# leavesnight/VIEO_SLAM

Measured on AMD Instinct MI355X. Metric: frontend+localBA frames/sec on EuRoC MH05 stereo-VIO; ATE vs ref, higher is better.
Workload: dtype u8 (extract/match) + f64 (pose optimisation)

## Files before the change

### vieo_slam_amd/csrc/lba.hip

```cpp
#include <atomic>
#include <chrono>
#include <mutex>
#include <thread>
#include <vector>

#include "gba_sparse_plan.h"
#include "imu_device.h"
#include "rccl_dl.h"

namespace vieo {

struct LbaKf {
  double p[3], qw, qx, qy, qz;
  int col;
  int fixed;
  double v[3], dbg[3], dba[3], bg[3], ba[3];
};

struct LbaImu {
  int i, j;
  int has_imu, robust;
  double InfoI[81];
  double infoBg, infoBa;
  vieo_imu_preint M;
// ... 29 lines not shown
  int np, n_free, npv;
  int pd;
  int n_imu;
  const LbaImu* imu;
  const int *kf_in, *kf_out;
  double* Ae;
  double *gchi0, *gchi;
  double* bfull;
  double* red;
  double* red_sc;
  const unsigned char* close;
  double thMono, thMonoClose, thStereo;
  double gw[3];
  double th_dist_far;
  double qRbe[4], pbe[3];
  int ldS;
  int* kf_list;
  int* kf_act;
  const int *kf_edge_first, *kf_edge_idx;
  int* tab;
  LbaKf *kf, *kf_bak;
  double *X, *X_bak;
  double* err;
  unsigned char *level, *erase, *mp_act;
  const int *mp_first, *mp_count;
  double* CB;
  double* Bs;
  double* Sp;
  size_t sp_stride;
  int ksplit;
  double *Hll, *bl, *Hpp, *bp, *Hs, *bs, *xp;
  unsigned char* occ;
  int use_occ;
  double *Hb, *Wp;
  int* big_fail;
  int nb;
  double *part0, *part, *part_m, *pmax;
  double* part_t;
  int* tail_cnt;
  int n_chunks;
  int fold_kernel;
  int *chunk_first, *chunk_kf;
  int* chunk_cnt;
  double* chunk_part;
  CamD cam;
  CamD cams[4];
  int n_cams;
  const unsigned char* ocam;
  double dMono, dStereo;
  int solver;
  int scale_opt;
  double* scl;
  double* sc_sys;
  double* psc;
  const int *sch_ptr, *sch_i, *sch_j, *sch_diag, *sch_off;
  int n_sch_diag, n_sch_off;
  const int *col_ptr, *tile_i, *tile_j;
  const int *row_ptr, *row_j, *row_tile;
  const int *upd_ptr, *upd;
  int nt, n_tiles;
};

__device__ __forceinline__ double win_scale(const LbaDev& D) { return D.scale_opt ? D.scl[0] : 1.0; }
__device__ __forceinline__ void scaled_point(const LbaDev& D, int m, double* Xs) {
  const double s = win_scale(D);
  Xs[0] = D.X[3 * (size_t)m] * s, Xs[1] = D.X[3 * (size_t)m + 1] * s, Xs[2] = D.X[3 * (size_t)m + 2] * s;
// ... 653 lines not shown
  }
  if (threadIdx.x == 0) out[w].lambda = 1e-5 * s_m[0];
}

typedef double double4_t __attribute__((ext_vector_type(4)));
static const int kChunkLm = 16, kLd = 3 * kChunkLm + 2;
#ifndef VIEO_SCHUR_AB
#define VIEO_SCHUR_AB 0
#endif

__global__ void __launch_bounds__(256)
k_lba_occ(const LbaDev* __restrict__ devs, const WinCtl* __restrict__ ctl) {
  const int w = blockIdx.y;
  if (!(ctl[w].flags & LBA_BEGIN)) return;
  const LbaDev& D = devs[w];
  if (!D.use_occ) return;
  const int np = D.npv, CB = (np + 64) >> 6, nchunks = (D.n_mp + kChunkLm - 1) / kChunkLm;
  const int e = blockIdx.x * 256 + threadIdx.x;
  if (np == 0 || e >= CB * nchunks) return;
  const int bi = e / nchunks, ch = e - bi * nchunks;
  const int a0 = bi * 64 / 6, a1 = min((bi * 64 + 63) / 6, D.n_free - 1);
  int any = D.scale_opt && (np - 1) >= bi * 64 && (np - 1) < bi * 64 + 64;
  for (int a = a0; a <= a1 && !any; a++)
    for (int j = 0; j < kChunkLm; j++) {
      const int m = ch * kChunkLm + j;
      if (m < D.n_mp && D.tab[(size_t)a * D.n_mp + m] >= 0) {
        any = 1;
        break;
      }
    }
  D.occ[e] = (unsigned char)any;
}

template <bool OFFDIAG, bool TILES = false>
__global__ void __launch_bounds__(256, OFFDIAG ? 2 : 3)
k_lba_schur(const LbaDev* __restrict__ devs, const WinCtl* __restrict__ ctl, const WinOut* __restrict__ out) {
  __shared__ __attribute__((aligned(16))) double sT[64 * kLd];
  __shared__ __attribute__((aligned(16))) double sB[64 * kLd];
  __shared__ double sDi[2][kChunkLm * 9];
  const int w = blockIdx.y;
  if (!(ctl[w].flags & LBA_TRIAL)) return;
  const LbaDev& D = devs[w];
  const int np = D.npv;
  if (np == 0) return;
  const int RB = (np + 63) >> 6, CB = (np + 64) >> 6;
  const int ksplit = D.ksplit;
  int bt = blockIdx.x / ksplit;
  const int split = blockIdx.x % ksplit;
  int bi = 0, bj;
  if (TILES != (D.solver == 3)) return;
  if (TILES) {
    if (bt >= (OFFDIAG ? D.n_sch_off : D.n_sch_diag)) return;
    bt = (OFFDIAG ? D.sch_off : D.sch_diag)[bt];
    bi = D.sch_i[bt], bj = D.sch_j[bt];
  } else if (OFFDIAG) {
    while (bi < RB && bt >= CB - bi - 1) bt -= CB - bi - 1, bi++;
    if (bi >= RB) return;
    bj = bi + 1 + bt;
  } else {
    if (bt >= RB) return;
    bi = bj = bt;
  }
  const int nchunks = (D.n_mp + kChunkLm - 1) / kChunkLm, cps = (nchunks + ksplit - 1) / ksplit;
  const int c0 = split * cps, c1 = min(nchunks, c0 + cps);
  if (c0 >= c1) return;
  const double lambda = win_lambda(ctl[w], out[w]);
  const int tid = threadIdx.x, lane = tid & 63;
  const int wv = __builtin_amdgcn_readfirstlane(tid >> 6);
  const int n_mp = D.n_mp;
  double4_t acc[4];
#pragma unroll
  for (int q = 0; q < 4; q++) acc[q] = (double4_t){0, 0, 0, 0};
  const unsigned char* occ_i = D.occ + (size_t)bi * nchunks;
  const unsigned char* occ_j = D.occ + (size_t)bj * nchunks;
  const bool has_bl = np >= bj * 64 && np < bj * 64 + 64;
  const bool use_occ = D.use_occ != 0;
  auto next_chunk = [&](int ch) {
    if (use_occ)
      while (ch < c1 && (!occ_i[ch] || (!has_bl && !occ_j[ch]))) ch++;
    return ch;
  };
  typedef double dbl2_t __attribute__((ext_vector_type(2)));
  typedef const dbl2_t __attribute__((address_space(1)))* gd2p;
  typedef const double __attribute__((address_space(1)))* gdp;
  typedef const int __attribute__((address_space(1)))* gip;
  typedef const unsigned char __attribute__((address_space(1)))* gbp;
  const gd2p gCB = (gd2p)D.CB;
  const gdp gBs = (gdp)D.Bs, gbl = (gdp)D.bl, gHll = (gdp)D.Hll;
  const gip gtab = (gip)D.tab;
  const gbp gact = (gbp)D.mp_act;
  const int ps = tid >> 4, pj = tid & 15;
  const int nfree = D.n_free, n_obs = D.n_obs;
  const bool sc_opt = D.scale_opt != 0;
  constexpr bool offdiag = OFFDIAG;
  const int aT = (64 * bi) / 6 + ps, aB = (64 * bj) / 6 + ps;
// ... 40 lines not shown
    if (lane < kChunkLm) {
#pragma unroll
      for (int t = 0; t < 9; t++) sDi[buf][lane * 9 + t] = hl_on ? Di[t] : 0.0;
    }
  };
  auto stage_T = [&](const double* v, const double* Di) {
    const double d0 = Di[0], d1 = Di[1], d2 = Di[2], d3 = Di[3], d4 = Di[4], d5 = Di[5], d6 = Di[6], d7 = Di[7], d8 = Di[8];
#pragma unroll
    for (int q = 0; q < 6; q++) {
      const unsigned r = (unsigned)(rT + q);
      if (r < 64u) {
        double b0 = v[3 * q], b1 = v[3 * q + 1], b2 = v[3 * q + 2];
        if (q == 0) b0 += spT3[0], b1 += spT3[1], b2 += spT3[2];
        double* d = sT + r * kLd + 3 * pj;
        d[0] = __builtin_fma(b2, d6, __builtin_fma(b1, d3, b0 * d0));
        d[1] = __builtin_fma(b2, d7, __builtin_fma(b1, d4, b0 * d1));
        d[2] = __builtin_fma(b2, d8, __builtin_fma(b1, d5, b0 * d2));
      }
    }
  };
  auto stage_B = [&](const double* v, const double* sp) {
#pragma unroll
    for (int q = 0; q < 6; q++) {
      const unsigned r = (unsigned)(rB + q);
      if (r < 64u) {
        double* d = sB + r * kLd + 3 * pj;
        double b0 = v[3 * q], b1 = v[3 * q + 1], b2 = v[3 * q + 2];
        if (q == 0) b0 += sp[0], b1 += sp[1], b2 += sp[2];
        if (q < 2 && (q == 1) == sc_opt) b0 += blv[0], b1 += blv[1], b2 += blv[2];
        d[0] = b0, d[1] = b1, d[2] = b2;
      }
    }
  };
#ifdef VIEO_SCHUR_PROBE
  long long tp[6] = {0, 0, 0, 0, 0, 0}, t0 = __builtin_readcyclecounter(), t1;
#define SCHUR_TICK(i) t1 = __builtin_readcyclecounter(), tp[i] += t1 - t0, t0 = t1;
#else
#define SCHUR_TICK(i)
#endif
  int ch = next_chunk(c0), buf = 0;
  int nx = ch < c1 ? next_chunk(ch + 1) : c1;
  int nx2 = nx < c1 ? next_chunk(nx + 1) : c1;
  int eT = -1, eB = -1;
  if (wv < 3) {
    load_blk(tab_of(aT, aTc, ch), ta);
    if (offdiag) load_blk(tab_of(aB, aBc, ch), tb);
    if (spT) load_special(aT, ch, !offdiag, spT3, blv);
    if (offdiag && spB) load_special(aB, ch, true, spB3, blv);
    eT = tab_of(aT, aTc, nx);
    if (offdiag) eB = tab_of(aB, aBc, nx);
  } else {
    load_hll(ch);
    store_dinv(0);
    load_hll(nx);
  }
  while (ch < c1) {
    __syncthreads();
    SCHUR_TICK(0)
    if (wv < 3) {
      if (!(VIEO_SCHUR_AB & 2)) {
        stage_T(ta, sDi[buf] + pj * 9);
        if (offdiag)
          stage_B(tb, spB3);
        else
          stage_B(ta, spT3);
      }
    } else {
      store_dinv(buf ^ 1);
      load_hll(nx2);
    }
    SCHUR_TICK(1)
    __syncthreads();
    SCHUR_TICK(2)
    const int nx3 = nx2 < c1 ? next_chunk(nx2 + 1) : c1;
    if (wv < 3 && nx < c1) {
      load_blk(eT, ta);
      if (offdiag) load_blk(eB, tb);
      if (spT) load_special(aT, nx, !offdiag, spT3, blv);
      if (offdiag && spB) load_special(aB, nx, true, spB3, blv);
      eT = tab_of(aT, aTc, nx2);
      if (offdiag) eB = tab_of(aB, aBc, nx2);
    }
    SCHUR_TICK(3)
    {
      const double* pa = sT + (wv * 16 + (lane & 15)) * kLd + (lane >> 4);
      const double* pb = sB + (lane & 15) * kLd + (lane >> 4);
#if !(VIEO_SCHUR_AB & 1)
#pragma unroll
      for (int ks = 0; ks < 3 * kChunkLm / 4; ks++) {
        const double av = pa[ks * 4];
#pragma unroll
        for (int q = 0; q < 4; q++)
          acc[q] = __builtin_amdgcn_mfma_f64_16x16x4f64(av, pb[q * 16 * kLd + ks * 4], acc[q], 0, 0, 0);
      }
#else
      acc[0][0] += pa[0] + pb[0];
#endif
    }
    SCHUR_TICK(4)
    buf ^= 1, ch = nx, nx = nx2, nx2 = nx3;
  }
#ifdef VIEO_SCHUR_PROBE
  if ((blockIdx.x == 3 || blockIdx.x == 40) && (blockIdx.y == 0 || blockIdx.y == 3) && (tid == 0 || tid == 64 || tid == 200))
    printf("schur probe w %d bx %d tid %d tile (%d,%d) chunks %d: wait_A %lld stage %lld wait_B %lld issue_loads %lld mfma %lld\n",
           w, (int)blockIdx.x, tid, bi, bj, c1 - c0, tp[0], tp[1], tp[2], tp[3], tp[4]);
#endif
  double* S = D.Sp + (size_t)split * D.sp_stride;
  if (TILES) {
    S += (size_t)bt * kGbaTileElems;
#pragma unroll
    for (int q = 0; q < 4; q++)
#pragma unroll
      for (int r = 0; r < 4; r++) S[(wv * 16 + (lane >> 4) + 4 * r) * 64 + q * 16 + (lane & 15)] = acc[q][r];
    return;
  }
#pragma unroll
  for (int q = 0; q < 4; q++)
#pragma unroll
    for (int r = 0; r < 4; r++)
      S[(size_t)(bi * 64 + wv * 16 + (lane >> 4) + 4 * r) * D.ldS + bj * 64 + q * 16 + (lane & 15)] = acc[q][r];
}

__global__ void __launch_bounds__(256)
k_lba_pack(const LbaDev* __restrict__ devs, const WinCtl* __restrict__ ctl) {
  const int w = blockIdx.y;
  if (!(ctl[w].flags & LBA_TRIAL)) return;
  const LbaDev& D = devs[w];
  if (!D.red) return;
  const int npv = D.npv, nS = npv * (npv + 1), nH = 36 * D.n_free, nb = 6 * D.n_free;
  const int e = blockIdx.x * 256 + threadIdx.x;
  if (e >= nS + nH + nb + (D.scale_opt ? nb + 2 : 0)) return;
  if (e < nS) {
    const int ksplit = D.ksplit;
    const int nchunks = (D.n_mp + kChunkLm - 1) / kChunkLm, cps = (nchunks + ksplit - 1) / ksplit;
    const int ns = (nchunks + cps - 1) / cps;
    const int r = e / (npv + 1), c = e - r * (npv + 1);
    const int rr = c < npv ? min(r, c) : r, cc = c < npv ? max(r, c) : npv;
    double s = 0;
    for (int k = 0; k < ns; k++) s += D.Sp[(size_t)k * D.sp_stride + (size_t)rr * D.ldS + cc];
    D.red[e] = s;
  } else if (e < nS + nH)
    D.red[e] = D.Hpp[e - nS];
  else if (e < nS + nH + nb)
    D.red[e] = D.bp[e - nS - nH];
  else
    D.red[e] = D.sc_sys[e - nS - nH - nb];
}

// ... 1543 lines not shown
    o.scl = take(16);
    H.o_kf = o.kf, H.o_X = o.X, H.o_erase = o.erase, H.o_scl = o.scl;
  }
  const size_t res_end = arena;
  for (int w = 0; w < W; w++) {
    const WinHost& H = win[w];
    if (H.skip) continue;
    off[w].level = take(H.n_obs), off[w].err = take((size_t)H.n_obs * 24);
  }
  const size_t zero_end = arena;
  if ((rc = g_stage.ensure(res_end)) != VIEO_OK) return rc;
  uint8_t* hs = (uint8_t*)g_stage.p;
  int max_obs = 0, max_mp = 0, max_kf = 0, max_nf = 0, max_imu = 0, max_chunks = 1;
  bool any_multicam = false;
  for (int w = 0; w < W; w++) {
    if (win[w].skip) continue;
    max_nf = std::max(max_nf, win[w].nf), max_mp = std::max(max_mp, win[w].n_mp);
  }
  const int cps_target = 8;
  auto schur_tiles = [&](int nf) {
    const int npm = 6 * nf + sco, RB = (npm + 63) / 64, CB = (npm + 64) / 64;
    return RB * CB - RB * (RB - 1) / 2;
  };
  auto schur_ksplit = [&](int nf, int nmp) {
    const int nch = (nmp + kChunkLm - 1) / kChunkLm, nbt = std::max(1, schur_tiles(nf));
    if (gba) return std::max(1, std::min(std::min(nch, 16), 768 / nbt));
    return std::max(1, std::min(std::min((nch + cps_target - 1) / cps_target, 32), std::max(1, 512 / nbt)));
  };
  int schur_grid = 0, schur_grid_off = 0;
  int schur_grid_t = 0, schur_grid_t_off = 0;
  std::vector<size_t> scratch_off(W);
  struct Scr {
    size_t kf_bak, X_bak, mp_act, BB, Bs, Sp, Hll, bl, Hpp, Hs, bp, bs, xp, part0, part, part_m, pmax, kf_list, tab, Ae, gchi0,
        gchi, bfull, Hb, Wp, big_fail, kf_act, occ, sc_sys, psc, part_t, tail_cnt, chunk_first, chunk_kf, chunk_cnt, chunk_part;
    int nb;
  };
  std::vector<Scr> scr(W);
  for (int w = 0; w < W; w++) {
    WinHost& H = win[w];
    if (H.skip) continue;
    const int nf = H.nf;
    Scr& s = scr[w];
    const int npm = 6 * nf + sco;
    s.kf_bak = take((size_t)H.n_kf * sizeof(LbaKf)), s.X_bak = take((size_t)H.n_mp * 24);
    s.mp_act = take(H.n_mp);
    const int sp_rows = (npm + 63) / 64 * 64, ldS = (npm + 64) / 64 * 64;
    s.BB = take(((size_t)H.n_obs + 1) * 144);
    s.Bs = sco ? take((size_t)std::max(H.n_mp, 1) * 24) : 0;
    const int ksplit = schur_ksplit(nf, H.n_mp);
    const bool tiles = wcls[w] == 3;
    const GbaSparsePlan& PL = plans[w];
    if (tiles) {
      schur_grid_t = std::max(schur_grid_t, (int)PL.sch_diag.size() * ksplit);
      schur_grid_t_off = std::max(schur_grid_t_off, (int)PL.sch_off.size() * ksplit);
    } else {
      const int RBw = (npm + 63) / 64;
      schur_grid = std::max(schur_grid, RBw * ksplit);
      schur_grid_off = std::max(schur_grid_off, (schur_tiles(nf) - RBw) * ksplit);
    }
    s.Sp = take(tiles ? PL.schur_bytes(ksplit) : (size_t)ksplit * sp_rows * ldS * 8);
    s.Hll = take((size_t)H.n_mp * 72), s.bl = take((size_t)H.n_mp * 24);
    const int npf = pd * nf + sco;
    s.Hpp = take((size_t)std::max(nf, 1) * 36 * 8), s.Hs = tiles ? 0 : take((size_t)npf * npf * 8);
    s.nb = (npf + 1 + kNB - 1) / kNB * kNB;
    s.Hb = s.Wp = s.big_fail = 0;
    if (tiles) {
      s.Hb = take(PL.pool_bytes()), s.Wp = take(PL.panel_bytes()), s.big_fail = take(256);
    } else if (wcls[w] == 2) {
      s.Hb = take((size_t)s.nb * s.nb * 8), s.Wp = take((size_t)s.nb * kNB * 8), s.big_fail = take(256);
    } else if (wcls[w] == 1) {
      s.nb = (npf + 16) >> 4;
      s.Hb = take(ldg_scratch_doubles(s.nb) * 8);
    }
    s.bp = take((size_t)npm * 8), s.bs = take((size_t)npf * 8), s.xp = take((size_t)npf * 8);
    s.bfull = take((size_t)npf * 8);
    s.Ae = take((size_t)std::max(H.n_imu, 1) * 930 * 8);
    s.gchi0 = take((size_t)std::max(H.n_imu, 1) * 8), s.gchi = take((size_t)std::max(H.n_imu, 1) * 8);
    s.part0 = take((size_t)((H.n_obs + 255) / 256) * 8), s.part = take((size_t)((H.n_obs + 255) / 256) * 8);
    s.part_m = take((size_t)((H.n_mp + 63) / 64) * 8), s.pmax = take((size_t)((H.n_mp + 63) / 64) * 8);
    s.part_t = take((size_t)std::max((H.n_mp + 63) / 64, 1) * 8), s.tail_cnt = take(256);
    {
      const size_t nchk = (size_t)H.n_obs / kBuildChunk + nf + 1;
      s.chunk_first = take((size_t)(nf + 1) * 4), s.chunk_cnt = take((size_t)(nf + 1) * 4);
      s.chunk_kf = take(nchk * 4), s.chunk_part = take(nchk * 33 * 8);
      max_chunks = std::max(max_chunks, (int)nchk);
    }
    s.kf_list = take((size_t)H.n_kf * 4), s.tab = take((size_t)std::max(nf, 1) * H.n_mp * 4);
    s.sc_sys = take((size_t)(6 * nf + 2) * 8), s.psc = take((size_t)((H.n_mp + 63) / 64) * 16);
    s.kf_act = take((size_t)H.n_kf * 4);
    s.occ = take((size_t)((npm + 64) / 64) * ((H.n_mp + kChunkLm - 1) / kChunkLm));
    LbaDev& D = devs[w];
    memset(&D, 0, sizeof(D));
    D.n_obs = H.n_obs, D.n_mp = H.n_mp, D.n_kf = H.n_kf, D.nf_cap = nf;
    D.ldS = ldS, D.sp_stride = tiles ? PL.n_sch_tiles() * kGbaTileElems : (size_t)sp_rows * ldS, D.ksplit = ksplit;
    D.cam.fx = H.P->fx, D.cam.fy = H.P->fy, D.cam.cx = H.P->cx, D.cam.cy = H.P->cy, D.cam.bf = H.P->bf;
    memcpy(D.cam.Rcb, H.P->Rcb, 72);
    memcpy(D.cam.tcb, H.P->tcb, 24);
    D.n_cams = H.P->n_cams;
    any_multicam |= H.P->n_cams > 0;
    for (int ci = 0; ci < H.P->n_cams; ci++) {
      const vieo_camera& c = H.P->cams[ci];
      CamD& d = D.cams[ci];
      d.fx = c.fx, d.fy = c.fy, d.cx = c.cx, d.cy = c.cy, d.bf = 0;
      memcpy(d.Rcb, c.Rcb, 72), memcpy(d.tcb, c.tcb, 24);
      d.model = c.model, d.num_k = c.model == VIEO_CAM_RADTAN ? c.num_k : 0;
      for (int q = 0; q < 8; q++) d.k[q] = (double)c.dist[q];
    }
    D.dMono = (double)(float)sqrt(gba ? 5.99 : 5.991), D.dStereo = (double)(float)sqrt(7.815);
    D.pd = pd, D.n_imu = H.n_imu;
    D.scale_opt = sco;
    D.use_occ = gba ? 1 : 0;
    D.solver = wcls[w];
    if (tiles) {
      D.n_sch_diag = (int)PL.sch_diag.size(), D.n_sch_off = (int)PL.sch_off.size();
      D.nt = PL.nt, D.n_tiles = (int)PL.n_tiles();
    }
    if (vio) {
      D.thMono = (double)5.991f, D.thMonoClose = 1.5 * (double)5.991f, D.thStereo = 7.815;
      memcpy(D.gw, H.VP->gw, 24);
      memcpy(D.qRbe, H.VP->qRbe, 32), memcpy(D.pbe, H.VP->pbe, 24);
      D.th_dist_far = (!gba && H.VP->th_dist_far > 0 && std::isfinite(H.VP->th_dist_far)) ? (double)H.VP->th_dist_far : 0.0;
      H.prelevel_pending = !gba;
    } else {
// ... 171 lines not shown
      g_lba_sparse_stats[0] = (long long)P.n_tiles(), g_lba_sparse_stats[1] = (long long)P.nt * (P.nt + 1) / 2;
      g_lba_sparse_stats[2] = (long long)P.n_sch_tiles(), g_lba_sparse_stats[3] = (long long)P.vrb * P.vcb - (long long)P.vrb * (P.vrb - 1) / 2;
      g_lba_sparse_stats[4] = (long long)P.bytes(devs[w].ksplit), g_lba_sparse_stats[5] = (long long)arena;
    }
  if ((rc = g_small.ensure(small_bytes)) != VIEO_OK) return rc;
  if ((rc = g_small_h.ensure((size_t)W * (sizeof(WinCtl) + sizeof(WinOut) + 32))) != VIEO_OK) return rc;
  uint8_t* base = g_arena.as<uint8_t>();
  for (int w = 0; w < W; w++) {
    if (win[w].skip) continue;
    const Off& o = off[w];
    const Scr& s = scr[w];
    LbaDev& D = devs[w];
    D.obs = (const vieo_lba_obs*)(base + o.obs);
    D.mp_first = (const int*)(base + o.mp_first), D.mp_count = (const int*)(base + o.mp_count);
    D.kf_edge_first = (const int*)(base + o.kf_edge_first), D.kf_edge_idx = (const int*)(base + o.kf_edge_idx);
    D.kf = (LbaKf*)(base + o.kf), D.X = (double*)(base + o.X), D.erase = base + o.erase;
    D.level = base + o.level, D.err = (double*)(base + o.err);
    D.ocam = base + o.ocam;
    D.kf_bak = (LbaKf*)(base + s.kf_bak), D.X_bak = (double*)(base + s.X_bak), D.mp_act = base + s.mp_act;
    D.CB = (double*)(base + s.BB), D.Bs = (double*)(base + s.Bs), D.Sp = (double*)(base + s.Sp);
    D.Hll = (double*)(base + s.Hll), D.bl = (double*)(base + s.bl);
    D.Hpp = (double*)(base + s.Hpp), D.Hs = (double*)(base + s.Hs), D.bp = (double*)(base + s.bp);
    D.Hb = (double*)(base + s.Hb), D.Wp = (double*)(base + s.Wp), D.big_fail = (int*)(base + s.big_fail);
    D.nb = s.nb;
    D.bs = (double*)(base + s.bs), D.xp = (double*)(base + s.xp);
    D.part0 = (double*)(base + s.part0), D.part = (double*)(base + s.part);
    D.part_m = (double*)(base + s.part_m), D.pmax = (double*)(base + s.pmax);
    D.part_t = (double*)(base + s.part_t), D.tail_cnt = (int*)(base + s.tail_cnt);
    D.fold_kernel = W <= 4 ? 0 : 1;
    D.chunk_first = (int*)(base + s.chunk_first), D.chunk_cnt = (int*)(base + s.chunk_cnt);
    D.chunk_kf = (int*)(base + s.chunk_kf), D.chunk_part = (double*)(base + s.chunk_part);
    D.kf_list = (int*)(base + s.kf_list), D.tab = (int*)(base + s.tab);
    D.kf_act = (int*)(base + s.kf_act), D.occ = base + s.occ;
    D.bfull = (double*)(base + s.bfull), D.Ae = (double*)(base + s.Ae);
    D.gchi0 = (double*)(base + s.gchi0), D.gchi = (double*)(base + s.gchi);
    D.scl = (double*)(base + o.scl), D.sc_sys = (double*)(base + s.sc_sys), D.psc = (double*)(base + s.psc);
    if (vio || win[w].ENC) {
      D.imu = (const LbaImu*)(base + o.imu), D.close = base + o.close;
      D.kf_in = (const int*)(base + o.kf_in), D.kf_out = (const int*)(base + o.kf_out);
    }
    if (wcls[w] == 3) {
      const int* d = (const int*)(base + o.plan);
      for (auto& l : plan_lists(plans[w], &D)) *l.second = d, d += l.first->size();
    }
  }
  size_t shard_sys = 0;
  if (sh) {
    for (int w = 0; w < W; w++) {
      if (win[w].skip) continue;
      devs[w].red = sh->d_buf + shard_sys;
      shard_sys += shard_sys_doubles(devs[w].nf_cap, sco);
    }
    if (shard_sys + 4 * (size_t)W > sh->cap) {
      set_error("sharded local BA: reduction buffer too small (%zu doubles needed)", shard_sys + 4 * (size_t)W);
      return VIEO_E_CAPACITY;
    }
    for (int w = 0; w < W; w++) devs[w].red_sc = sh->d_buf + shard_sys + 4 * (size_t)w;
  }
  LbaDev* dD = g_small.as<LbaDev>();
  WinCtl* dC = (WinCtl*)(dD + W);
  WinOut* dO = (WinOut*)(dC + W);
  int* dWins = (int*)(dO + W);
  WinCtl* ctl = (WinCtl*)g_small_h.p;
  WinOut* out = (WinOut*)(ctl + W);
  double* h_sc = (double*)(out + W);
  const double ms_described = ms_since(t_enter);
// ... 79 lines not shown
          H.stage = 2;
        else if (H.stage == 0 && !stop_now) {
          f |= LBA_CLASS0;
          H.stage = 1, H.iters = H.P->its1, H.phase = H.iters > 0 ? 0 : 2;
        } else {
          if (H.stage == 0) H.R->status = VIEO_LBA_ABORTED;
          f |= LBA_CLASS1;
          H.stage = 2;
        }
      }
      if (H.stage < 2 && H.phase == 0) {
        f |= LBA_BEGIN | LBA_BUILD | LBA_TRIAL | ((gba ? gba->robust != 0 : H.stage == 0) ? LBA_ROBUST : 0);
        lam = vio && !gba ? H.VP->lambda_init : -1;
        if (H.prelevel_pending) f |= LBA_PRELEVEL, H.prelevel_pending = false;
      } else if (H.stage < 2 && H.phase == 1) {
        f |= LBA_TRIAL | ((gba ? gba->robust != 0 : H.stage == 0) ? LBA_ROBUST : 0);
        if (H.need_build) f |= LBA_BUILD;
        if (H.need_restore) f |= LBA_RESTORE, H.need_restore = false;
      }
      ctl[w].flags = f, ctl[w].pad = sh ? stop_req : 0, ctl[w].lambda = lam;
      any |= f;
      if ((f & LBA_TRIAL) && !H.skip) cls_trial[devs[w].solver] = true;
    }
    if (!any) break;
    VIEO_HIP_CHECK(hipMemcpyAsync(dC, ctl, (size_t)W * sizeof(WinCtl), hipMemcpyHostToDevice, st));
    if (any & LBA_RESTORE) KT.launch(KC_OTHER, [&] { hipLaunchKernelGGL(k_lba_restore, dim3(gr, W), dim3(256), 0, st, dD, dC); });
    if (any & (LBA_CLASS0 | LBA_CLASS1)) KT.launch(KC_OTHER, [&] { hipLaunchKernelGGL(k_lba_classify, dim3(ge, W), dim3(256), 0, st, dD, dC); });
    if (any & LBA_PRELEVEL)
      for (int ph = 0; ph < 3; ph++) KT.launch(KC_OTHER, [&] { hipLaunchKernelGGL(k_lba_prelevel, dim3(ge, W), dim3(256), 0, st, dD, dC, ph); });
    if (any & LBA_BEGIN) {
      KT.launch(KC_BEGIN, [&] { hipLaunchKernelGGL(k_lba_zero, dim3(64, W), dim3(256), 0, st, dD, dC); });
      KT.launch(KC_BEGIN, [&] { hipLaunchKernelGGL(k_lba_begin, dim3(W), dim3(1024), 0, st, dD, dC, dO); });
      if (gba) KT.launch(KC_BEGIN, [&] { hipLaunchKernelGGL(k_lba_occ, dim3(std::max(1, (occ_max + 255) / 256), W), dim3(256), 0, st, dD, dC); });
      KT.launch(KC_ERROR, [&] { hipLaunchKernelGGL(k_lba_error, dim3(ge, W), dim3(256), 0, st, dD, dC, 0); });
    }
    if (any & LBA_BUILD) {
      auto build2 = [&](auto mc, auto sc) {
        constexpr bool MC = decltype(mc)::value, SC = decltype(sc)::value;
        if (fused_build) {
          KT.launch(KC_BUILD, [&] { hipLaunchKernelGGL((k_lba_build<MC, SC, 2>), dim3(gq + max_chunks + max_imu, W), dim3(256), 0, st, dD, dC, max_chunks, gq); });
          if (W > 4) KT.launch(KC_BUILD, [&] { hipLaunchKernelGGL(k_lba_build_fold, dim3(std::max(1, max_nf), W), dim3(64), 0, st, dD, dC); });
          return;
        }
        KT.launch(KC_BUILD, [&] { hipLaunchKernelGGL((k_lba_build<MC, SC, 0>), dim3(gq, W), dim3(256), 0, st, dD, dC, 0, 0); });
        KT.launch(KC_BUILD, [&] { hipLaunchKernelGGL((k_lba_build<MC, SC, 1>), dim3(max_chunks, W), dim3(256), 0, st, dD, dC, max_chunks, 0); });
        if (W > 4) KT.launch(KC_BUILD, [&] { hipLaunchKernelGGL(k_lba_build_fold, dim3(std::max(1, max_nf), W), dim3(64), 0, st, dD, dC); });
      };
      if (sco) {
        if (any_multicam)
          build2(std::true_type(), std::true_type());
        else
          build2(std::false_type(), std::true_type());
        KT.launch(KC_BUILD, [&] { hipLaunchKernelGGL(k_lba_scale_fold, dim3(W), dim3(256), 0, st, dD, dC); });
      } else if (any_multicam)
        build2(std::true_type(), std::false_type());
      else
        build2(std::false_type(), std::false_type());
      if (!fused_build && max_imu > 0) KT.launch(KC_GENERIC, [&] { hipLaunchKernelGGL(k_lba_generic, dim3(max_imu, W), dim3(64), 0, st, dD, dC, 0); });
    }
    if (any & LBA_BEGIN) KT.launch(KC_BEGIN, [&] { hipLaunchKernelGGL(k_lba_lambda, dim3(W), dim3(256), 0, st, dD, dC, dO); });
    if (any & LBA_TRIAL) {
      if (dense_wins) {
        KT.launch(KC_SCHUR, [&] { hipLaunchKernelGGL(k_lba_schur<false>, dim3(std::max(1, schur_grid), W), dim3(256), 0, st, dD, dC, dO); });
        if (schur_grid_off > 0)
          KT.launch(KC_SCHUR, [&] { hipLaunchKernelGGL(k_lba_schur<true>, dim3(schur_grid_off, W), dim3(256), 0, st, dD, dC, dO); });
      }
      if (sparse && cls_trial[3]) {
        KT.launch(KC_SCHUR, [&] { hipLaunchKernelGGL((k_lba_schur<false, true>), dim3(std::max(1, schur_grid_t), W), dim3(256), 0, st, dD, dC, dO); });
        if (schur_grid_t_off > 0)
          KT.launch(KC_SCHUR, [&] { hipLaunchKernelGGL((k_lba_schur<true, true>), dim3(schur_grid_t_off, W), dim3(256), 0, st, dD, dC, dO); });
      }
      if (sh) {
        KT.launch(KC_OTHER, [&] { hipLaunchKernelGGL(k_lba_pack, dim3((unsigned)((shard_sys_doubles(max_nf, sco) + 255) / 256), W), dim3(256), 0, st,
                           dD, dC); });
        if ((rc = shard_exchange(sh, sh->d_buf, shard_sys, st)) != VIEO_OK) return rc;
      }
      for (int c = 0; c < 3; c++) {
        const int nw = cls_first[c + 1] - cls_first[c];
        if (nw <= 0 || !cls_trial[c]) continue;
        const unsigned gx = (unsigned)(((size_t)cls_max[c] * cls_max[c] + 255) / 256);
        KT.launch(KC_ASSEMBLE, [&] { hipLaunchKernelGGL(k_lba_assemble, dim3(gx, nw), dim3(256), 0, st, dD, dC, dO, dWins + cls_first[c]); });
      }
      if (big && cls_trial[2]) {
        const int nbm = (n_max_b + 1 + kNB - 1) / kNB * kNB, ntm = nbm / kNB;
        KT.launch(KC_LDLT, [&] { hipLaunchKernelGGL(k_big_init, dim3((unsigned)(((size_t)nbm * nbm + 255) / 256), W), dim3(256), 0, st, dD, dC); });
        for (int k = 0; k < ntm; k++) {
          const int below = nbm - (k + 1) * kNB, m = ntm - k - 1;
          KT.launch(KC_LDLT, [&] { hipLaunchKernelGGL(k_big_panel<false>, dim3(1 + (below + 255) / 256, W), dim3(256), 0, st, dD, dC, k); });
          if (m > 0) KT.launch(KC_LDLT, [&] { hipLaunchKernelGGL(k_big_syrk<false>, dim3(m * (m + 1) / 2, W), dim3(256), 0, st, dD, dC, k); });
        }
        for (int sb = 0; sb < (n_max_b + kNB - 1) / kNB; sb++)
          KT.launch(KC_LDLT, [&] { hipLaunchKernelGGL(k_big_back_step<false>, dim3(1 + (n_max_b + 255) / 256, W), dim3(256), 0, st, dD, dC, sb); });
        KT.launch(KC_LDLT, [&] { hipLaunchKernelGGL(k_big_finish<false>, dim3(W), dim3(256), 0, st, dD, dC, dO); });
      }
      if (sparse && cls_trial[3]) {
        const int nw = cls_first[4] - cls_first[3];
        const unsigned ga = (unsigned)std::min<size_t>(16384, std::max<size_t>(1, (sp_elems + 255) / 256));
        KT.launch(KC_ASSEMBLE, [&] { hipLaunchKernelGGL(k_lba_assemble_tiles, dim3(ga, nw), dim3(256), 0, st, dD, dC, dO, dWins + cls_first[3]); });
        for (int k = 0; k < sp_nt; k++) {
          KT.launch(KC_LDLT_SPARSE, [&] { hipLaunchKernelGGL(k_big_panel<true>, dim3(sp_panel_grid[k], W), dim3(256), 0, st, dD, dC, k); });
          if (sp_syrk_grid[k] > 0)
            KT.launch(KC_LDLT_SPARSE, [&] { hipLaunchKernelGGL(k_big_syrk<true>, dim3(sp_syrk_grid[k], W), dim3(256), 0, st, dD, dC, k); });
        }
// ... 365 lines not shown
```

Measured before the change: 59200.

## Stage dense Schur tiles from compacted per-chunk edge lists

Adds kernels that count, prefix-scan and fill a compact list of non-empty (keyframe slot, landmark) edge entries for each tile-row and landmark chunk, once per LBA begin. The dense Schur kernel then gathers only the existing camera-landmark blocks and scatters them into zeroed shared-memory tiles, instead of probing the dense tab for every slot. This cuts wasted global loads on sparse co-visibility. The cost is three extra launches, extra scratch memory, per-iteration shared-memory clears, and special-casing of the scale and bl rows. The tiled sparse path is split into its own kernel, k_lba_schur_tiles.

```diff
diff --git a/vieo_slam_amd/csrc/lba.hip b/vieo_slam_amd/csrc/lba.hip
--- a/vieo_slam_amd/csrc/lba.hip
+++ b/vieo_slam_amd/csrc/lba.hip
@@ -85,6 +85,8 @@
   double *Hll, *bl, *Hpp, *bp, *Hs, *bs, *xp;
   unsigned char* occ;
   int use_occ;
+  int* sl_ent;
+  int* sl_off;
   double *Hb, *Wp;
   int* big_fail;
   int nb;
@@ -804,9 +806,9 @@
   D.occ[e] = (unsigned char)any;
 }
 
-template <bool OFFDIAG, bool TILES = false>
+template <bool OFFDIAG>
 __global__ void __launch_bounds__(256, OFFDIAG ? 2 : 3)
-k_lba_schur(const LbaDev* __restrict__ devs, const WinCtl* __restrict__ ctl, const WinOut* __restrict__ out) {
+k_lba_schur_tiles(const LbaDev* __restrict__ devs, const WinCtl* __restrict__ ctl, const WinOut* __restrict__ out) {
   __shared__ __attribute__((aligned(16))) double sT[64 * kLd];
   __shared__ __attribute__((aligned(16))) double sB[64 * kLd];
   __shared__ double sDi[2][kChunkLm * 9];
@@ -815,24 +817,13 @@
   const LbaDev& D = devs[w];
   const int np = D.npv;
   if (np == 0) return;
-  const int RB = (np + 63) >> 6, CB = (np + 64) >> 6;
   const int ksplit = D.ksplit;
   int bt = blockIdx.x / ksplit;
   const int split = blockIdx.x % ksplit;
-  int bi = 0, bj;
-  if (TILES != (D.solver == 3)) return;
-  if (TILES) {
-    if (bt >= (OFFDIAG ? D.n_sch_off : D.n_sch_diag)) return;
-    bt = (OFFDIAG ? D.sch_off : D.sch_diag)[bt];
-    bi = D.sch_i[bt], bj = D.sch_j[bt];
-  } else if (OFFDIAG) {
-    while (bi < RB && bt >= CB - bi - 1) bt -= CB - bi - 1, bi++;
-    if (bi >= RB) return;
-    bj = bi + 1 + bt;
-  } else {
-    if (bt >= RB) return;
-    bi = bj = bt;
-  }
+  if (D.solver != 3) return;
+  if (bt >= (OFFDIAG ? D.n_sch_off : D.n_sch_diag)) return;
+  bt = (OFFDIAG ? D.sch_off : D.sch_diag)[bt];
+  const int bi = D.sch_i[bt], bj = D.sch_j[bt];
   const int nchunks = (D.n_mp + kChunkLm - 1) / kChunkLm, cps = (nchunks + ksplit - 1) / ksplit;
   const int c0 = split * cps, c1 = min(nchunks, c0 + cps);
   if (c0 >= c1) return;
@@ -939,12 +930,6 @@
       }
     }
   };
-#ifdef VIEO_SCHUR_PROBE
-  long long tp[6] = {0, 0, 0, 0, 0, 0}, t0 = __builtin_readcyclecounter(), t1;
-#define SCHUR_TICK(i) t1 = __builtin_readcyclecounter(), tp[i] += t1 - t0, t0 = t1;
-#else
-#define SCHUR_TICK(i)
-#endif
   int ch = next_chunk(c0), buf = 0;
   int nx = ch < c1 ? next_chunk(ch + 1) : c1;
   int nx2 = nx < c1 ? next_chunk(nx + 1) : c1;
@@ -963,7 +948,6 @@
   }
   while (ch < c1) {
     __syncthreads();
-    SCHUR_TICK(0)
     if (wv < 3) {
       if (!(VIEO_SCHUR_AB & 2)) {
         stage_T(ta, sDi[buf] + pj * 9);
@@ -976,9 +960,7 @@
       store_dinv(buf ^ 1);
       load_hll(nx2);
     }
-    SCHUR_TICK(1)
     __syncthreads();
-    SCHUR_TICK(2)
     const int nx3 = nx2 < c1 ? next_chunk(nx2 + 1) : c1;
     if (wv < 3 && nx < c1) {
       load_blk(eT, ta);
@@ -988,6 +970,373 @@
       eT = tab_of(aT, aTc, nx2);
       if (offdiag) eB = tab_of(aB, aBc, nx2);
     }
+    {
+      const double* pa = sT + (wv * 16 + (lane & 15)) * kLd + (lane >> 4);
+      const double* pb = sB + (lane & 15) * kLd + (lane >> 4);
+#if !(VIEO_SCHUR_AB & 1)
+#pragma unroll
+      for (int ks = 0; ks < 3 * kChunkLm / 4; ks++) {
+        const double av = pa[ks * 4];
+#pragma unroll
+        for (int q = 0; q < 4; q++)
+          acc[q] = __builtin_amdgcn_mfma_f64_16x16x4f64(av, pb[q * 16 * kLd + ks * 4], acc[q], 0, 0, 0);
+      }
+#else
+      acc[0][0] += pa[0] + pb[0];
+#endif
+    }
+    buf ^= 1, ch = nx, nx = nx2, nx2 = nx3;
+  }
+  double* S = D.Sp + (size_t)split * D.sp_stride + (size_t)bt * kGbaTileElems;
+#pragma unroll
+  for (int q = 0; q < 4; q++)
+#pragma unroll
+    for (int r = 0; r < 4; r++) S[(wv * 16 + (lane >> 4) + 4 * r) * 64 + q * 16 + (lane & 15)] = acc[q][r];
+}
+
+static const int kSlotsPerTile = 12, kPairsPerUnit = kSlotsPerTile * kChunkLm;
+static const int kSlEdgeBits = 24;
+template <bool FILL>
+__global__ void __launch_bounds__(256)
+k_lba_schur_list(const LbaDev* __restrict__ devs, const WinCtl* __restrict__ ctl) {
+  const int w = blockIdx.y;
+  if (!(ctl[w].flags & LBA_BEGIN)) return;
+  const LbaDev& D = devs[w];
+  if (D.solver == 3) return;
+  const int np = D.npv, nchunks = (D.n_mp + kChunkLm - 1) / kChunkLm, units = ((np + 64) >> 6) * nchunks;
+  const int u = blockIdx.x * 4 + (threadIdx.x >> 6), lane = threadIdx.x & 63;
+  if (np == 0 || u >= units) return;
+  const int bi = u / nchunks, ch = u - bi * nchunks;
+  const int base = FILL ? D.sl_off[u] : 0;
+  int total = 0;
+  for (int k = 0; k < kPairsPerUnit / 64; k++) {
+    const int pr = k * 64 + lane, a = (64 * bi) / 6 + (pr >> 4), m = ch * kChunkLm + (pr & 15);
+    int e = -1;
+    if (a < D.n_free && 6 * a - 64 * bi < 64 && m < D.n_mp) e = D.tab[(size_t)a * D.n_mp + m];
+    const unsigned long long mask = __ballot(e >= 0);
+    if (FILL && e >= 0) D.sl_ent[base + total + __popcll(mask & ((1ull << lane) - 1))] = e | (pr << kSlEdgeBits);
+    total += __popcll(mask);
+  }
+  if (!FILL && lane == 0) D.sl_off[u] = total;
+}
+
+__global__ void __launch_bounds__(1024)
+k_lba_schur_list_scan(const LbaDev* __restrict__ devs, const WinCtl* __restrict__ ctl) {
+  __shared__ int s_sum[1024];
+  const int w = blockIdx.x, tid = threadIdx.x;
+  if (!(ctl[w].flags & LBA_BEGIN)) return;
+  const LbaDev& D = devs[w];
+  if (D.solver == 3) return;
+  const int np = D.npv, nchunks = (D.n_mp + kChunkLm - 1) / kChunkLm, units = np == 0 ? 0 : ((np + 64) >> 6) * nchunks;
+  const int seg = (units + 1023) / 1024, u0 = min(units, tid * seg), u1 = min(units, u0 + seg);
+  int sum = 0;
+  for (int u = u0; u < u1; u++) sum += D.sl_off[u];
+  s_sum[tid] = sum;
+  __syncthreads();
+  for (int o = 1; o < 1024; o <<= 1) {
+    const int v = tid >= o ? s_sum[tid - o] : 0;
+    __syncthreads();
+    s_sum[tid] += v;
+    __syncthreads();
+  }
+  int run = s_sum[tid] - sum;
+  for (int u = u0; u < u1; u++) {
+    const int c = D.sl_off[u];
+    D.sl_off[u] = run, run += c;
+  }
+  if (tid == 1023) D.sl_off[units] = s_sum[1023];
+}
+
+template <int N, class F>
+__device__ __forceinline__ void schur_passes(F&& f) {
+  if constexpr (N > 0) {
+    schur_passes<N - 1>(f);
+    f(std::integral_constant<int, N - 1>());
+  }
+}
+
+template <bool OFFDIAG>
+__global__ void __launch_bounds__(256, OFFDIAG ? 2 : 3)
+k_lba_schur(const LbaDev* __restrict__ devs, const WinCtl* __restrict__ ctl, const WinOut* __restrict__ out) {
+  __shared__ __attribute__((aligned(16))) double sT[64 * kLd];
+  __shared__ __attribute__((aligned(16))) double sB[64 * kLd];
+  __shared__ double sDi[2][kChunkLm * 9];
+  const int w = blockIdx.y;
+  if (!(ctl[w].flags & LBA_TRIAL)) return;
+  const LbaDev& D = devs[w];
+  const int np = D.npv;
+  if (np == 0 || D.solver == 3) return;
+  const int RB = (np + 63) >> 6, CB = (np + 64) >> 6;
+  const int ksplit = D.ksplit;
+  int bt = blockIdx.x / ksplit;
+  const int split = blockIdx.x % ksplit;
+  int bi = 0, bj;
+  if (OFFDIAG) {
+    while (bi < RB && bt >= CB - bi - 1) bt -= CB - bi - 1, bi++;
+    if (bi >= RB) return;
+    bj = bi + 1 + bt;
+  } else {
+    if (bt >= RB) return;
+    bi = bj = bt;
+  }
+  const int nchunks = (D.n_mp + kChunkLm - 1) / kChunkLm, cps = (nchunks + ksplit - 1) / ksplit;
+  const int c0 = split * cps, c1 = min(nchunks, c0 + cps);
+  if (c0 >= c1) return;
+  const double lambda = win_lambda(ctl[w], out[w]);
+  const int tid = threadIdx.x, lane = tid & 63;
+  const int wv = __builtin_amdgcn_readfirstlane(tid >> 6);
+  const int n_mp = D.n_mp;
+  double4_t acc[4];
+#pragma unroll
+  for (int q = 0; q < 4; q++) acc[q] = (double4_t){0, 0, 0, 0};
+  const unsigned char* occ_i = D.occ + (size_t)bi * nchunks;
+  const unsigned char* occ_j = D.occ + (size_t)bj * nchunks;
+  const bool has_bl = np >= bj * 64 && np < bj * 64 + 64;
+  const bool use_occ = D.use_occ != 0;
+  auto next_chunk = [&](int ch) {
+    if (use_occ)
+      while (ch < c1 && (!occ_i[ch] || (!has_bl && !occ_j[ch]))) ch++;
+    return ch;
+  };
+  typedef double dbl2_t __attribute__((ext_vector_type(2)));
+  typedef const dbl2_t __attribute__((address_space(1)))* gd2p;
+  typedef const double __attribute__((address_space(1)))* gdp;
+  typedef const int __attribute__((address_space(1)))* gip;
+  typedef const unsigned char __attribute__((address_space(1)))* gbp;
+  const gd2p gCB = (gd2p)D.CB;
+  const gdp gBs = (gdp)D.Bs, gbl = (gdp)D.bl, gHll = (gdp)D.Hll;
+  const gip goff = (gip)D.sl_off, gent = (gip)D.sl_ent;
+  const gbp gact = (gbp)D.mp_act;
+  const int ps = tid >> 4, pj = tid & 15;
+  const int nfree = D.n_free;
+  const bool sc_opt = D.scale_opt != 0;
+  constexpr bool offdiag = OFFDIAG;
+  const int s0T = (64 * bi) / 6, s0B = (64 * bj) / 6;
+  const int aT = s0T + ps, aB = s0B + ps;
+  const int rT = 6 * aT - 64 * bi, rB = 6 * aB - 64 * bj;
+  const bool spT = wv < 3 && nfree >= s0T + 4 * wv && nfree < s0T + 4 * wv + 4;
+  const bool spB = wv < 3 && nfree >= s0B + 4 * wv && nfree < s0B + 4 * wv + 4;
+  auto load_special = [&](int a, int ch, bool with_bl, double* sp, double* blv, bool& mine, unsigned char& act) {
+    const int m = ch * kChunkLm + pj, mc = min(m, n_mp - 1);
+    mine = a == nfree && m < n_mp && ch < c1;
+    if (sc_opt) sp[0] = gBs[3 * (size_t)mc], sp[1] = gBs[3 * (size_t)mc + 1], sp[2] = gBs[3 * (size_t)mc + 2];
+    if (with_bl) {
+      blv[0] = gbl[3 * (size_t)mc], blv[1] = gbl[3 * (size_t)mc + 1], blv[2] = gbl[3 * (size_t)mc + 2];
+      act = gact[mc];
+    }
+  };
+  double spT3[3] = {0, 0, 0}, spB3[3] = {0, 0, 0}, blv[3] = {0, 0, 0}, hl[3];
+  bool mineT = false, mineB = false, hl_in = false;
+  unsigned char bl_act = 0, hl_on = 0;
+  auto load_hll = [&](int ch) {
+#pragma unroll
+    for (int t = 0; t < 3; t++) hl[t] = gHll[min(ch * (kChunkLm * 9) + t * 64 + lane, 9 * n_mp - 1)];
+    const int m = ch * kChunkLm + (lane & 15);
+    hl_in = ch < c1 && m < n_mp, hl_on = gact[min(m, n_mp - 1)];
+  };
+  auto store_dinv = [&](int buf) {
+#pragma unroll
+    for (int t = 0; t < 3; t++)
+      if (t * 64 + lane < kChunkLm * 9) sDi[buf][t * 64 + lane] = hl[t];
+    __builtin_amdgcn_wave_barrier();
+    if (lane < kChunkLm) {
+      double H[9], Di[9];
+#pragma unroll
+      for (int t = 0; t < 9; t++) H[t] = sDi[buf][lane * 9 + t];
+      landmark_dinv(H, lambda, Di);
+#pragma unroll
+      for (int t = 0; t < 9; t++) sDi[buf][lane * 9 + t] = (hl_in && hl_on) ? Di[t] : 0.0;
+    }
+  };
+  constexpr int kGath = 256 / 9, kPass = (kPairsPerUnit + kGath - 1) / kGath;
+  const int gk = tid / 9, gp = tid - 9 * gk;
+  const bool glane = gk < kGath;
+  const int gq0 = (2 * gp) / 3, gc0 = 2 * gp - 3 * gq0, gq1 = (2 * gp + 1) / 3, gc1 = 2 * gp + 1 - 3 * gq1;
+  const int blq = sc_opt ? 1 : 0;
+  struct Side {
+    dbl2_t blk[kPass];
+    unsigned pos[(kPass + 3) / 4];
+    int ent[kPass];
+    int nC, o1, n1;
+    int pa, pb;
+  };
+  auto issue_off = [&](Side& s, int tile, int c) {
+    const int u = tile * nchunks + min(c, nchunks - 1);
+    s.pa = goff[u], s.pb = goff[u + 1];
+  };
+  auto take_off = [&](const Side& s, int c, int& o, int& n) {
+    o = __builtin_amdgcn_readfirstlane(s.pa), n = __builtin_amdgcn_readfirstlane(c < c1 ? s.pb - s.pa : 0);
+  };
+  auto tiers = [&](int n, auto&& f) {
+    if (n > 4 * kGath)
+      schur_passes<kPass>(f);
+    else if (n > 2 * kGath)
+      schur_passes<4>(f);
+    else if (n > 0)
+      schur_passes<2>(f);
+  };
+  auto load_ent = [&](Side& s, int o, int n) {
+    tiers(n, [&](auto pc) {
+      constexpr int p = decltype(pc)::value;
+      s.ent[p] = gent[o + min(p * kGath + gk, n - 1)];
+    });
+  };
+  auto load_blk = [&](Side& s, int n) {
+    tiers(n, [&](auto pc) {
+      constexpr int p = decltype(pc)::value;
+      if (!(VIEO_SCHUR_AB & 4)) s.blk[p] = gCB[9 * (size_t)(s.ent[p] & ((1 << kSlEdgeBits) - 1)) + gp];
+      const unsigned pr = (unsigned)s.ent[p] >> kSlEdgeBits;
+      s.pos[p / 4] = p % 4 ? s.pos[p / 4] | pr << 8 * (p % 4) : pr;
+    });
+  };
+  auto scatter = [&](const Side& s, double* tile, int slot0, int tb, bool settle) {
+#pragma unroll
+    for (int p = 0; p < kPass; p++)
+      if (p * kGath < s.nC) {
+        const int idx = p * kGath + gk;
+        if (glane && idx < s.nC) {
+          const unsigned pr = s.pos[p / 4] >> 8 * (p % 4) & 255u;
+          const int r0 = 6 * (slot0 + (int)(pr >> 4)) - 64 * tb;
+          double* d = tile + 3 * (pr & 15);
+          double x0 = s.blk[p][0], x1 = s.blk[p][1];
+          if (settle && gq0 <= blq) x0 += 0.0;
+          if (settle && gq1 <= blq) x1 += 0.0;
+          if ((unsigned)(r0 + gq0) < 64u) d[(r0 + gq0) * kLd + gc0] = x0;
+          if ((unsigned)(r0 + gq1) < 64u) d[(r0 + gq1) * kLd + gc1] = x1;
+        }
+      }
+  };
+  Side sa, sb;
+#pragma unroll
+  for (int p = 0; p < kPass; p++) {
+    sa.blk[p] = sb.blk[p] = (dbl2_t){0, 0};
+    sa.pos[p / 4] = sb.pos[p / 4] = 0, sa.ent[p] = sb.ent[p] = 0;
+  }
+  sb.nC = sb.o1 = sb.n1 = sb.pa = sb.pb = 0;
+  int tposC = 0, tpos1 = 0;
+#ifdef VIEO_SCHUR_PROBE
+  long long tp[6] = {0, 0, 0, 0, 0, 0}, t0 = __builtin_readcyclecounter(), t1;
+#define SCHUR_TICK(i) t1 = __builtin_readcyclecounter(), tp[i] += t1 - t0, t0 = t1;
+#else
+#define SCHUR_TICK(i)
+#endif
+  int ch = next_chunk(c0), buf = 0;
+  int nx = ch < c1 ? next_chunk(ch + 1) : c1;
+  int nx2 = nx < c1 ? next_chunk(nx + 1) : c1;
+  auto prologue = [&](Side& s, int tile, int& o0) {
+    issue_off(s, tile, ch), take_off(s, ch, o0, s.nC);
+    issue_off(s, tile, nx), take_off(s, nx, s.o1, s.n1);
+    load_ent(s, o0, s.nC), load_blk(s, s.nC), load_ent(s, s.o1, s.n1);
+    issue_off(s, tile, nx2);
+  };
+  {
+    int o0;
+    prologue(sa, bi, o0);
+    tposC = (int)((unsigned)gent[o0 + min(tid, max(sa.nC, 1) - 1)] >> kSlEdgeBits);
+    if (offdiag) prologue(sb, bj, o0);
+  }
+  if (wv < 3) {
+    if (spT) load_special(aT, ch, !offdiag, spT3, blv, mineT, bl_act);
+    if (offdiag && spB) load_special(aB, ch, true, spB3, blv, mineB, bl_act);
+  } else {
+    load_hll(ch);
+    store_dinv(0);
+    load_hll(nx);
+  }
+  dbl2_t* const sT2 = (dbl2_t*)sT + wv * (16 * kLd / 2);
+  auto clear_own_T = [&]() {
+#pragma unroll
+    for (int i = 0; i < (16 * kLd / 2 + 63) / 64; i++)
+      if (i * 64 + lane < 16 * kLd / 2) sT2[i * 64 + lane] = (dbl2_t){0, 0};
+  };
+  clear_own_T();
+  while (ch < c1) {
+    __syncthreads();
+    SCHUR_TICK(0)
+    if (!(VIEO_SCHUR_AB & 2)) {
+#pragma unroll
+      for (int i = 0; i < (64 * kLd / 2 + 255) / 256; i++)
+        if (i * 256 + tid < 64 * kLd / 2) ((dbl2_t*)sB)[i * 256 + tid] = (dbl2_t){0, 0};
+      scatter(sa, sT, s0T, bi, false);
+    }
+    if (wv == 3) {
+      store_dinv(buf ^ 1);
+      load_hll(nx2);
+    }
+    __syncthreads();
+    if (!(VIEO_SCHUR_AB & 2)) {
+      if (offdiag) scatter(sb, sB, s0B, bj, true);
+      if (tid < sa.nC) {
+        const int lm = tposC & 15, r0 = 6 * (s0T + (tposC >> 4)) - 64 * bi;
+        const double* Di = sDi[buf] + lm * 9;
+        const double d0 = Di[0], d1 = Di[1], d2 = Di[2], d3 = Di[3], d4 = Di[4], d5 = Di[5], d6 = Di[6], d7 = Di[7], d8 = Di[8];
+#pragma unroll
+        for (int q = 0; q < 6; q++) {
+          const unsigned r = (unsigned)(r0 + q);
+          if (r < 64u) {
+            double* d = sT + r * kLd + 3 * lm;
+            double b0 = d[0], b1 = d[1], b2 = d[2];
+            if (q == 0) b0 += 0.0, b1 += 0.0, b2 += 0.0;
+            d[0] = __builtin_fma(b2, d6, __builtin_fma(b1, d3, b0 * d0));
+            d[1] = __builtin_fma(b2, d7, __builtin_fma(b1, d4, b0 * d1));
+            d[2] = __builtin_fma(b2, d8, __builtin_fma(b1, d5, b0 * d2));
+            if (!offdiag) {
+              if (q == 1 && sc_opt) b0 += 0.0, b1 += 0.0, b2 += 0.0;
+              double* e = sB + r * kLd + 3 * lm;
+              e[0] = b0, e[1] = b1, e[2] = b2;
+            }
+          }
+        }
+      }
+      if (spT && aT == nfree) {
+        const bool on = mineT && sc_opt;
+        const double b0 = 0.0 + (on ? spT3[0] : 0.0), b1 = 0.0 + (on ? spT3[1] : 0.0), b2 = 0.0 + (on ? spT3[2] : 0.0);
+        if ((unsigned)rT < 64u) {
+          const double* Di = sDi[buf] + pj * 9;
+          double* d = sT + rT * kLd + 3 * pj;
+          d[0] = __builtin_fma(b2, Di[6], __builtin_fma(b1, Di[3], b0 * Di[0]));
+          d[1] = __builtin_fma(b2, Di[7], __builtin_fma(b1, Di[4], b0 * Di[1]));
+          d[2] = __builtin_fma(b2, Di[8], __builtin_fma(b1, Di[5], b0 * Di[2]));
+        }
+      }
+      if ((offdiag ? spB : spT) && aB == nfree) {
+        const double* sp = offdiag ? spB3 : spT3;
+        const bool mine = offdiag ? mineB : mineT, on = mine && sc_opt, onb = mine && bl_act != 0;
+        const double bl3[3] = {onb ? blv[0] : 0.0, onb ? blv[1] : 0.0, onb ? blv[2] : 0.0};
+        double v0[3] = {0.0 + (on ? sp[0] : 0.0), 0.0 + (on ? sp[1] : 0.0), 0.0 + (on ? sp[2] : 0.0)};
+        if (!sc_opt) v0[0] += bl3[0], v0[1] += bl3[1], v0[2] += bl3[2];
+        if ((unsigned)rB < 64u) {
+          double* d = sB + rB * kLd + 3 * pj;
+          d[0] = v0[0], d[1] = v0[1], d[2] = v0[2];
+        }
+        if (sc_opt && (unsigned)(rB + 1) < 64u) {
+          double* d = sB + (rB + 1) * kLd + 3 * pj;
+          d[0] = 0.0 + bl3[0], d[1] = 0.0 + bl3[1], d[2] = 0.0 + bl3[2];
+        }
+      }
+    }
+    SCHUR_TICK(1)
+    __syncthreads();
+    SCHUR_TICK(2)
+    const int nx3 = nx2 < c1 ? next_chunk(nx2 + 1) : c1;
+    {
+      int o2, n2, o2b = 0, n2b = 0;
+      take_off(sa, nx2, o2, n2);
+      if (offdiag) take_off(sb, nx2, o2b, n2b);
+      load_blk(sa, sa.n1), load_ent(sa, o2, n2);
+      tpos1 = (int)((unsigned)gent[sa.o1 + min(tid, max(sa.n1, 1) - 1)] >> kSlEdgeBits);
+      issue_off(sa, bi, nx3);
+      sa.nC = sa.n1, sa.o1 = o2, sa.n1 = n2;
+      if (offdiag) {
+        load_blk(sb, sb.n1), load_ent(sb, o2b, n2b);
+        issue_off(sb, bj, nx3);
+        sb.nC = sb.n1, sb.o1 = o2b, sb.n1 = n2b;
+      }
+    }
+    if (wv < 3 && nx < c1) {
+      if (spT) load_special(aT, nx, !offdiag, spT3, blv, mineT, bl_act);
+      if (offdiag && spB) load_special(aB, nx, true, spB3, blv, mineB, bl_act);
+    }
     SCHUR_TICK(3)
     {
       const double* pa = sT + (wv * 16 + (lane & 15)) * kLd + (lane >> 4);
@@ -1004,8 +1353,9 @@
       acc[0][0] += pa[0] + pb[0];
 #endif
     }
+    clear_own_T();
     SCHUR_TICK(4)
-    buf ^= 1, ch = nx, nx = nx2, nx2 = nx3;
+    buf ^= 1, ch = nx, nx = nx2, nx2 = nx3, tposC = tpos1;
   }
 #ifdef VIEO_SCHUR_PROBE
   if ((blockIdx.x == 3 || blockIdx.x == 40) && (blockIdx.y == 0 || blockIdx.y == 3) && (tid == 0 || tid == 64 || tid == 200))
@@ -1013,14 +1363,6 @@
            w, (int)blockIdx.x, tid, bi, bj, c1 - c0, tp[0], tp[1], tp[2], tp[3], tp[4]);
 #endif
   double* S = D.Sp + (size_t)split * D.sp_stride;
-  if (TILES) {
-    S += (size_t)bt * kGbaTileElems;
-#pragma unroll
-    for (int q = 0; q < 4; q++)
-#pragma unroll
-      for (int r = 0; r < 4; r++) S[(wv * 16 + (lane >> 4) + 4 * r) * 64 + q * 16 + (lane & 15)] = acc[q][r];
-    return;
-  }
 #pragma unroll
   for (int q = 0; q < 4; q++)
 #pragma unroll
@@ -2630,7 +2972,7 @@
   std::vector<size_t> scratch_off(W);
   struct Scr {
     size_t kf_bak, X_bak, mp_act, BB, Bs, Sp, Hll, bl, Hpp, Hs, bp, bs, xp, part0, part, part_m, pmax, kf_list, tab, Ae, gchi0,
-        gchi, bfull, Hb, Wp, big_fail, kf_act, occ, sc_sys, psc, part_t, tail_cnt, chunk_first, chunk_kf, chunk_cnt, chunk_part;
+        gchi, bfull, Hb, Wp, big_fail, kf_act, occ, sl_off, sl_ent, sc_sys, psc, part_t, tail_cnt, chunk_first, chunk_kf, chunk_cnt, chunk_part;
     int nb;
   };
   std::vector<Scr> scr(W);
@@ -2687,6 +3029,12 @@
     s.sc_sys = take((size_t)(6 * nf + 2) * 8), s.psc = take((size_t)((H.n_mp + 63) / 64) * 16);
     s.kf_act = take((size_t)H.n_kf * 4);
     s.occ = take((size_t)((npm + 64) / 64) * ((H.n_mp + kChunkLm - 1) / kChunkLm));
+    s.sl_off = take(tiles ? 4 : ((size_t)((npm + 64) / 64) * ((H.n_mp + kChunkLm - 1) / kChunkLm) + 1) * 4);
+    s.sl_ent = take(tiles ? 8 : (size_t)std::max(H.n_obs, 1) * (nf > 10 ? 2 : 1) * 4 + 4);
+    if (!tiles && H.n_obs >= (1 << kSlEdgeBits)) {
+      set_error("local BA: window %d has %d observations, the Schur staging's lists index %d", w, H.n_obs, 1 << kSlEdgeBits);
+      return VIEO_E_CAPACITY;
+    }
     LbaDev& D = devs[w];
     memset(&D, 0, sizeof(D));
     D.n_obs = H.n_obs, D.n_mp = H.n_mp, D.n_kf = H.n_kf, D.nf_cap = nf;
@@ -2924,6 +3272,7 @@
     D.chunk_kf = (int*)(base + s.chunk_kf), D.chunk_part = (double*)(base + s.chunk_part);
     D.kf_list = (int*)(base + s.kf_list), D.tab = (int*)(base + s.tab);
     D.kf_act = (int*)(base + s.kf_act), D.occ = base + s.occ;
+    D.sl_off = (int*)(base + s.sl_off), D.sl_ent = (int*)(base + s.sl_ent);
     D.bfull = (double*)(base + s.bfull), D.Ae = (double*)(base + s.Ae);
     D.gchi0 = (double*)(base + s.gchi0), D.gchi = (double*)(base + s.gchi);
     D.scl = (double*)(base + o.scl), D.sc_sys = (double*)(base + s.sc_sys), D.psc = (double*)(base + s.psc);
@@ -3069,6 +3418,12 @@
       KT.launch(KC_BEGIN, [&] { hipLaunchKernelGGL(k_lba_zero, dim3(64, W), dim3(256), 0, st, dD, dC); });
       KT.launch(KC_BEGIN, [&] { hipLaunchKernelGGL(k_lba_begin, dim3(W), dim3(1024), 0, st, dD, dC, dO); });
       if (gba) KT.launch(KC_BEGIN, [&] { hipLaunchKernelGGL(k_lba_occ, dim3(std::max(1, (occ_max + 255) / 256), W), dim3(256), 0, st, dD, dC); });
+      if (dense_wins) {
+        const dim3 gl(std::max(1, (occ_max + 3) / 4), W);
+        KT.launch(KC_BEGIN, [&] { hipLaunchKernelGGL(k_lba_schur_list<false>, gl, dim3(256), 0, st, dD, dC); });
+        KT.launch(KC_BEGIN, [&] { hipLaunchKernelGGL(k_lba_schur_list_scan, dim3(W), dim3(1024), 0, st, dD, dC); });
+        KT.launch(KC_BEGIN, [&] { hipLaunchKernelGGL(k_lba_schur_list<true>, gl, dim3(256), 0, st, dD, dC); });
+      }
       KT.launch(KC_ERROR, [&] { hipLaunchKernelGGL(k_lba_error, dim3(ge, W), dim3(256), 0, st, dD, dC, 0); });
     }
     if (any & LBA_BUILD) {
@@ -3103,9 +3458,9 @@
           KT.launch(KC_SCHUR, [&] { hipLaunchKernelGGL(k_lba_schur<true>, dim3(schur_grid_off, W), dim3(256), 0, st, dD, dC, dO); });
       }
       if (sparse && cls_trial[3]) {
-        KT.launch(KC_SCHUR, [&] { hipLaunchKernelGGL((k_lba_schur<false, true>), dim3(std::max(1, schur_grid_t), W), dim3(256), 0, st, dD, dC, dO); });
+        KT.launch(KC_SCHUR, [&] { hipLaunchKernelGGL(k_lba_schur_tiles<false>, dim3(std::max(1, schur_grid_t), W), dim3(256), 0, st, dD, dC, dO); });
         if (schur_grid_t_off > 0)
-          KT.launch(KC_SCHUR, [&] { hipLaunchKernelGGL((k_lba_schur<true, true>), dim3(schur_grid_t_off, W), dim3(256), 0, st, dD, dC, dO); });
+          KT.launch(KC_SCHUR, [&] { hipLaunchKernelGGL(k_lba_schur_tiles<true>, dim3(schur_grid_t_off, W), dim3(256), 0, st, dD, dC, dO); });
       }
       if (sh) {
         KT.launch(KC_OTHER, [&] { hipLaunchKernelGGL(k_lba_pack, dim3((unsigned)((shard_sys_doubles(max_nf, sco) + 255) / 256), W), dim3(256), 0, st,
```

Result: no change. 58970 (-0.4%).
